# simone7monaco/NO-NODE-comparison

Hardware: NVIDIA B200
Metric: train trajectories/s (EGNO 20-body, fwd+bwd+Adam) (higher is better)
Workload: dtype f32

## Files before the change

include/nbody_b200.h:

```cpp
#ifndef NBODY_B200_H
#define NBODY_B200_H

#include <stdint.h>

#ifdef __cplusplus
extern "C" {
#endif

#define NB_HIDDEN 64
#define NB_MAX_EDGE_FEA 4
#define NB_MAX_T 16
#define NB_MAX_NODES 100

#define NB_OK 0
#define NB_ERR_INVALID (-1)
#define NB_ERR_CUDA (-2)

typedef struct NbEgnoConfig {
  int32_t B;
  int32_t N;
  int32_t T;
  int32_t n_layers;
  int32_t num_modes;
  int32_t in_node_nf;
  int32_t in_edge_nf;
  int32_t time_emb_dim;
  int32_t use_time_conv;
  int32_t num_inputs;
} NbEgnoConfig;

typedef struct NbSegnoConfig {
  int32_t B;
  int32_t N;
  int32_t T;
  int32_t in_node_nf;
  int32_t in_edge_nf;
  int32_t recurrent;
  float coords_weight;
  int32_t h_given;
} NbSegnoConfig;

int nb_version(void);
const char* nb_last_error(void);

int64_t nb_egno_param_count(const NbEgnoConfig* cfg);
int64_t nb_segno_param_count(const NbSegnoConfig* cfg);

#define NB_WS_FORWARD_INFER 0
#define NB_WS_BACKWARD 1
#define NB_WS_FORWARD_TRAIN 2
int64_t nb_egno_saved_floats(const NbEgnoConfig* cfg);
int64_t nb_egno_workspace_floats(const NbEgnoConfig* cfg, int mode);
int64_t nb_segno_saved_floats(const NbSegnoConfig* cfg);
int64_t nb_segno_workspace_floats(const NbSegnoConfig* cfg, int mode);

int nb_egno_forward(const NbEgnoConfig* cfg, const float* params, const float* x, const float* nodes,
                    const float* edge_fea, const float* v, const float* loc_mean, const int64_t* timesteps_out,
                    const int64_t* timesteps_in, float* x_out, float* v_out, float* h_out, float* saved,
                    float* workspace, void* stream);

int nb_egno_backward(const NbEgnoConfig* cfg, const float* params, const float* nodes, const float* edge_fea,
                     const float* loc_mean, const int64_t* timesteps_out, const int64_t* timesteps_in,
                     const float* saved, const float* g_x_out, const float* g_v_out, const float* g_h_out,
                     float* grad_params, float* g_x_in, float* g_v_in, float* workspace, void* stream);

int nb_segno_forward(const NbSegnoConfig* cfg, const float* params, const float* his, const float* x, const float* v,
                     const float* edge_attr, float* x_out, float* h_out, float* v_out, float* saved,
                     float* workspace, void* stream);

int nb_segno_backward(const NbSegnoConfig* cfg, const float* params, const float* his, const float* edge_attr,
                      const float* saved, const float* g_x_out, const float* g_h_out, const float* g_v_out,
                      float* grad_params, float* g_x_in, float* g_v_in, float* g_h_in, float* workspace, void* stream);

int nb_segno_embed_forward(const NbSegnoConfig* cfg, const float* params, int64_t rows, const float* his, float* h,
                           void* stream);
int64_t nb_segno_embed_backward_workspace_floats(const NbSegnoConfig* cfg, int64_t rows);
int nb_segno_embed_backward(const NbSegnoConfig* cfg, int64_t rows, const float* his, const float* g_h, float* grad_params,
                            float* workspace, void* stream);
int nb_segno_merge_forward(int32_t mode, int64_t n, int32_t L, int32_t frame, const float* h_all, const float* x_all,
                           const float* v_all, const float* h_int, const float* x_int, const float* v_int,
                           const float* attn_params, float* h_out, float* x_out, float* v_out, float* alpha, void* stream);
int64_t nb_segno_merge_backward_workspace_floats(int64_t n);
int nb_segno_merge_backward(int32_t mode, int64_t n, int32_t L, int32_t frame, const float* h_all, const float* x_all,
                            const float* v_all, const float* h_int, const float* x_int, const float* v_int,
                            const float* attn_params, const float* alpha, const float* g_h, const float* g_x,
                            const float* g_v, float* g_h_all, float* g_x_all, float* g_v_all, float* g_h_int,
                            float* g_x_int, float* g_v_int, float* g_attn, int32_t accumulate, float* workspace,
                            void* stream);
int nb_accumulate(int64_t n, float* dst, const float* src, void* stream);

int nb_check_canonical_edges(const int64_t* row, const int64_t* col, int64_t n_edges, int32_t B, int32_t N,
                             int32_t* flag_dev, void* stream);


int nb_egcl_edge_forward(int32_t n_gt, int32_t B, int32_t N, int32_t n_edge_fea, int32_t clamp_per_edge,
                         const float* x, const float* P, const float* Q, const float* edge_fea, const float* w1,
                         int32_t ldw1, int32_t col_rad, int32_t col_ef, const float* W2, const float* b2,
                         const float* W3, const float* b3, const float* w4, const float* b4, float* M, float* Fsum,
                         void* stream);

int64_t nb_egcl_edge_backward_workspace_floats(int32_t n_gt, int32_t N);
int nb_egcl_edge_backward(int32_t n_gt, int32_t B, int32_t N, int32_t n_edge_fea, int32_t clamp_per_edge,
                          const float* x, const float* P, const float* Q, const float* edge_fea, const float* w1,
                          int32_t ldw1, int32_t col_rad, int32_t col_ef, const float* W2, const float* b2,
                          const float* W3, const float* b3, const float* w4, const float* b4, const float* gM,
                          const float* gFsum, float* gP, float* gQ, float* gx, float* gw, float* workspace,
                          void* stream);

long long nb_launch_count(void);
#define NB_PROFILE_CATEGORIES 8
int nb_profile_enable(int enable);
int nb_profile_read(double* ms , long long* counts );

int nb_set_edge_impl(int impl);
int nb_get_edge_impl(void);
int nb_set_node_impl(int impl);
int nb_get_node_impl(void);
int nb_set_node_fused(int on);
int nb_get_node_fused(void);
int nb_set_segno_fused(int on);
int nb_get_segno_fused(void);

int nb_nbody_features(int32_t B, int32_t N, int32_t with_charge, const float* loc, const float* vel, const float* charges,
                      const float* edge_attr_o, float* nodes, float* loc_mean, float* edge_attr, void* stream);
int nb_nbody_energy(int32_t kind, int32_t F, int32_t B, int32_t N, float G, const float* loc, const float* vel,
                    const float* charges, float* energy, void* stream);

int64_t nb_traj_mse_workspace_floats(int32_t T);
int nb_traj_mse(int32_t T, int64_t rows, int32_t target_layout, int32_t only_first, const float* pred, const float* target,
                float* losses, float* loss, float* grad, float* workspace, void* stream);

int nb_sim_charged(int32_t B, int32_t N, int32_t T, int32_t sample_freq, double dt, double strength, double max_force,
                   double box_size, const double* loc0, const double* vel0, const double* charges, double* loc, double* vel,
                   void* stream);
int nb_sim_gravity(int32_t B, int32_t N, int32_t T, int32_t sample_freq, double dt, double G, double softening,
                   const double* pos0, const double* vel0, const double* mass, double* pos, double* vel, double* force,
                   void* stream);

int nb_adam_step(int64_t n, float* params, const float* grads, float* exp_avg, float* exp_avg_sq, float* step,
                 int32_t tick, double lr, double beta1, double beta2, double eps, double weight_decay, double grad_scale,
                 void* stream);
int nb_adam_step_peers(int64_t n, float* params, const void* const* peer_grads, int32_t npeer, float* exp_avg,
                       float* exp_avg_sq, float* step, int32_t tick, double lr, double beta1, double beta2, double eps,
                       double weight_decay, double grad_scale, void* stream);

int nb_tc_selftest(int32_t mode, const float* A, const float* W, float* out, void* stream);

int nb_silu_selftest(int64_t n, const float* x, float* out_mufu, float* out_fma, void* stream);

#ifdef __cplusplus
}
#endif
#endif
```

no-node-comparison_b200/_cabi.py:

```python
from __future__ import annotations

import ctypes as C

c_f = C.c_void_p


class NbEgnoConfig(C.Structure):
    _fields_ = [("B", C.c_int32), ("N", C.c_int32), ("T", C.c_int32), ("n_layers", C.c_int32),
                ("num_modes", C.c_int32), ("in_node_nf", C.c_int32), ("in_edge_nf", C.c_int32),
                ("time_emb_dim", C.c_int32), ("use_time_conv", C.c_int32), ("num_inputs", C.c_int32)]


class NbSegnoConfig(C.Structure):
    _fields_ = [("B", C.c_int32), ("N", C.c_int32), ("T", C.c_int32), ("in_node_nf", C.c_int32),
                ("in_edge_nf", C.c_int32), ("recurrent", C.c_int32), ("coords_weight", C.c_float),
                ("h_given", C.c_int32)]


EXPORTS = {
    "nb_version": (C.c_int, []),
    "nb_last_error": (C.c_char_p, []),
    "nb_egno_param_count": (C.c_int64, [C.POINTER(NbEgnoConfig)]),
    "nb_segno_param_count": (C.c_int64, [C.POINTER(NbSegnoConfig)]),
    "nb_egno_saved_floats": (C.c_int64, [C.POINTER(NbEgnoConfig)]),
    "nb_egno_workspace_floats": (C.c_int64, [C.POINTER(NbEgnoConfig), C.c_int]),
    "nb_segno_saved_floats": (C.c_int64, [C.POINTER(NbSegnoConfig)]),
    "nb_segno_workspace_floats": (C.c_int64, [C.POINTER(NbSegnoConfig), C.c_int]),
    "nb_egno_forward": (C.c_int, [C.POINTER(NbEgnoConfig)] + [c_f] * 14),
    "nb_egno_backward": (C.c_int, [C.POINTER(NbEgnoConfig)] + [c_f] * 15),
    "nb_segno_forward": (C.c_int, [C.POINTER(NbSegnoConfig)] + [c_f] * 11),
    "nb_segno_backward": (C.c_int, [C.POINTER(NbSegnoConfig)] + [c_f] * 13),
    "nb_segno_embed_forward": (C.c_int, [C.POINTER(NbSegnoConfig), c_f, C.c_int64, c_f, c_f, c_f]),
    "nb_segno_embed_backward_workspace_floats": (C.c_int64, [C.POINTER(NbSegnoConfig), C.c_int64]),
    "nb_segno_embed_backward": (C.c_int, [C.POINTER(NbSegnoConfig), C.c_int64] + [c_f] * 5),
    "nb_segno_merge_forward": (C.c_int, [C.c_int32, C.c_int64, C.c_int32, C.c_int32] + [c_f] * 12),
    "nb_segno_merge_backward_workspace_floats": (C.c_int64, [C.c_int64]),
    "nb_segno_merge_backward": (C.c_int, [C.c_int32, C.c_int64, C.c_int32, C.c_int32] + [c_f] * 18 + [C.c_int32, c_f, c_f]),
    "nb_accumulate": (C.c_int, [C.c_int64, c_f, c_f, c_f]),
    "nb_check_canonical_edges": (C.c_int, [c_f, c_f, C.c_int64, C.c_int32, C.c_int32, c_f, c_f]),
    "nb_egcl_edge_forward": (C.c_int, [C.c_int32] * 5 + [c_f] * 5 + [C.c_int32] * 3 + [c_f] * 9),
    "nb_egcl_edge_backward_workspace_floats": (C.c_int64, [C.c_int32, C.c_int32]),
    "nb_egcl_edge_backward": (C.c_int, [C.c_int32] * 5 + [c_f] * 5 + [C.c_int32] * 3 + [c_f] * 14),
    "nb_nbody_features": (C.c_int, [C.c_int32] * 3 + [c_f] * 8),
    "nb_nbody_energy": (C.c_int, [C.c_int32] * 4 + [C.c_float] + [c_f] * 5),
    "nb_sim_charged": (C.c_int, [C.c_int32] * 4 + [C.c_double] * 4 + [c_f] * 6),
    "nb_sim_gravity": (C.c_int, [C.c_int32] * 4 + [C.c_double] * 3 + [c_f] * 7),
    "nb_traj_mse_workspace_floats": (C.c_int64, [C.c_int32]),
    "nb_traj_mse": (C.c_int, [C.c_int32, C.c_int64, C.c_int32, C.c_int32] + [c_f] * 7),
    "nb_adam_step": (C.c_int, [C.c_int64] + [c_f] * 5 + [C.c_int32] + [C.c_double] * 6 + [c_f]),
    "nb_adam_step_peers": (C.c_int, [C.c_int64, c_f, C.POINTER(C.c_void_p), C.c_int32] + [c_f] * 3 + [C.c_int32] + [C.c_double] * 6 + [c_f]),
    "nb_launch_count": (C.c_longlong, []),
    "nb_profile_enable": (C.c_int, [C.c_int]),
    "nb_profile_read": (C.c_int, [C.POINTER(C.c_double), C.POINTER(C.c_longlong)]),
    "nb_set_edge_impl": (C.c_int, [C.c_int]),
    "nb_set_node_impl": (C.c_int, [C.c_int]),
    "nb_get_node_impl": (C.c_int, []),
    "nb_set_node_fused": (C.c_int, [C.c_int]),
    "nb_get_node_fused": (C.c_int, []),
    "nb_set_segno_fused": (C.c_int, [C.c_int]),
    "nb_get_segno_fused": (C.c_int, []),
    "nb_get_edge_impl": (C.c_int, []),
    "nb_tc_selftest": (C.c_int, [C.c_int32, c_f, c_f, c_f, c_f]),
    "nb_silu_selftest": (C.c_int, [C.c_int64, c_f, c_f, c_f, c_f]),
}


def declare(lib: C.CDLL) -> C.CDLL:
    for name, (res, args) in EXPORTS.items():
        fn = getattr(lib, name)
        fn.restype = res
        fn.argtypes = args
    return lib
```

no-node-comparison_b200/csrc/nb_edge_sel.cuh:

```cuda
#pragma once
#ifndef NB_EMU
#include "nb_edge.cuh"
#include "nb_tc.cuh"
#include "nb_edge_tc.cuh"

#define NB_SEL_MAX_GN 27
#define NB_SEL_XC0 54

struct NbSelUnit {
  int R;
  int gt0;
  int recv0, nrecv;
  int send0, nsend;
  int RC;
  int I0, J0;
  bool first_j, last_j;
  bool first_i, last_i;
};
template <bool BLK>
__device__ __forceinline__ NbSelUnit nb_sel_unit(const NbEdgeGeom& g, int uo, int sub) {
  NbSelUnit U;
  if (!BLK) {
    U.gt0 = uo * g.G;
    const int ngt = min(g.G, g.NGT - U.gt0);
// ... 338 lines not shown
                 sNl = nb_smem_u32(Nl), sFh = nb_smem_u32(Fh), sFl = nb_smem_u32(Fl), sW2h = nb_smem_u32(W2h),
                 sW2l = nb_smem_u32(W2l), sW3h = nb_smem_u32(W3h), sW3l = nb_smem_u32(W3l);
  const float b4 = __ldg(a.w.b4);
  uint32_t phase = 0;

  const int n_outer = BLK ? g.NGT : g.n_units, n_sub = BLK ? g.nI * g.nJ : 1;
  for (int uo = blockIdx.x; uo < n_outer; uo += gridDim.x)
  for (int sub = 0; sub < n_sub; ++sub) {
    const NbSelUnit U = nb_sel_unit<BLK>(g, uo, sub);
    const int R = U.R;
    {
      const int n3r = U.nrecv * 3, n3 = n3r + (BLK ? U.nsend * 3 : 0);
      const int t_x = tid + (U.first_j ? 0 : n3r);
      float xv = 0.f;
      if (t_x < n3) xv = t_x < n3r ? __ldg(a.x + (int64_t)U.recv0 * 3 + t_x) : __ldg(a.x + (int64_t)U.send0 * 3 + (t_x - n3r));
      nb_sel_stage_unit(Nh, Nl, a.P, a.Q, U, tid, NB_THREADS, U.first_j);
      if (t_x < n3) {
        if (t_x < n3r) xs[t_x] = xv;
        else xq[t_x - n3r] = xv;
      }
    }
    const float* xsnd = BLK ? xq : xs;
    __syncthreads();

    for (int r0 = 0; r0 < R; r0 += NB_TILE) {
      float dx = 0.f, dy = 0.f, dz = 0.f, r2 = 0.f;
      float e[NB_MAX_EF];
#pragma unroll
      for (int f = 0; f < NB_MAX_EF; ++f) e[f] = 0.f;
      int li = 0, lj = 0, gt = 0, rem = 0;
      const bool valid = nb_sel_row<BLK>(g, U, rowinfo, r0 + row, li, lj, gt, rem);
      if (valid) {
        dx = xs[li * 3 + 0] - xsnd[lj * 3 + 0];
        dy = xs[li * 3 + 1] - xsnd[lj * 3 + 1];
        dz = xs[li * 3 + 2] - xsnd[lj * 3 + 2];
        r2 = dx * dx + dy * dy + dz * dz;
        const int64_t eoff = ((int64_t)nb_ef_graph(g, gt) * g.EPG + rem) * g.nef;
#pragma unroll
        for (int f = 0; f < NB_MAX_EF; ++f)
          if (f < g.nef) e[f] = __ldg(a.ef + eoff + f);
      }
      if (r0 > 0) {
        nb_mbar_wait(bar, phase);
        phase ^= 1;
        nb_tc_fence_after();
      }
      nb_sel_write_row(Sel, row, hf, valid, li, U.RC + lj, r2, e);
      nb_fence_async_smem();
      nb_tc_fence_before();
      __syncthreads();
      if (NB_ISSUER(0)) {
        nb_tc_fence_after();
        nb_issue_gather(tm, sSel, sNh, sNl, 4, idesc_gat, 0u);
        nb_mma_commit(bar);
      }
      nb_mbar_wait(bar, phase);
      phase ^= 1;
      nb_tc_fence_after();
      {
        float v[32];
        nb_tmem_ld32(tm_mine, v);
#pragma unroll
        for (int i = 0; i < 32; ++i) v[i] = NB_FWD_SILU(i, v[i]);
        nb_store32_ta(nullptr, nullptr, row, hf, v, ta_hm, ta_lm);
        nb_tmem_st_wait();
      }
      nb_tc_fence_before();
      __syncthreads();
      if (NB_ISSUER(0)) {
        nb_tc_fence_after();
        nb_issue_w3_ta(tm, ta_h, ta_l, sW2h, sW2l, false, idesc_fwd, 0u);
        nb_mma_commit(bar);
      }
      nb_mbar_wait(bar, phase);
      phase ^= 1;
      nb_tc_fence_after();
      {
        float v[32];
        nb_tmem_ld32(tm_mine, v);
#pragma unroll
        for (int i = 0; i < 32; ++i) v[i] = NB_FWD_SILU(i, v[i] + vb2[cb + i]);
        nb_store32_ta(Th, Tl, row, hf, v, ta_hm, ta_lm);
        nb_tmem_st_wait();
      }
      nb_fence_async_smem();
      nb_tc_fence_before();
      __syncthreads();
      if (NB_ISSUER(0)) {
        nb_tc_fence_after();
        nb_issue_w3_ta(tm, ta_h, ta_l, sW3h, sW3l, false, idesc_fwd, 0u);
        nb_mma_commit(bar);
        nb_issue_scatter(tm + 64, sSel, sTh, sTl, idesc_sc, (r0 > 0 || !U.first_j) ? 1u : 0u);
      }
      nb_mbar_wait(bar, phase);
      phase ^= 1;
      nb_tc_fence_after();
      {
        float v[32];
        nb_tmem_ld32(tm_mine, v);
        float cp = 0.f;
#pragma unroll
        for (int i = 0; i < 32; ++i) cp = fmaf(vw4[cb + i], NB_FWD_SILU(i, v[i] + vb3[cb + i]), cp);
        cpart[hf * NB_TILE + row] = cp;
      }
      nb_tc_fence_before();
      __syncthreads();
      if (hf == 0) {
        float c = cpart[row] + cpart[NB_TILE + row] + b4;
        float fx = dx * c, fy = dy * c, fz = dz * c;
        if (g.clamp_edge) {
          fx = fminf(fmaxf(fx, -100.f), 100.f);
          fy = fminf(fmaxf(fy, -100.f), 100.f);
          fz = fminf(fmaxf(fz, -100.f), 100.f);
        }
        const uint32_t px = nb_pack_split(fx), py = nb_pack_split(fy), pz = nb_pack_split(fz);
        *reinterpret_cast<uint4*>(Fh + row * 16) = make_uint4((px & 0xffffu) | (py << 16), pz & 0xffffu, 0u, 0u);
        *reinterpret_cast<uint4*>(Fl + row * 16) = make_uint4((px >> 16) | (py & 0xffff0000u), pz >> 16, 0u, 0u);
      }
      nb_fence_async_smem();
      __syncthreads();
      if (NB_ISSUER(0)) {
        nb_tc_fence_after();
        nb_issue_scatter8(tm + 128, sSel, sFh, sFl, idesc_sc8, (r0 > 0 || !U.first_j) ? 1u : 0u);
        nb_mma_commit(bar);
      }
    }
    nb_mbar_wait(bar, phase);
    phase ^= 1;
    nb_tc_fence_after();
    if (U.last_j) {
      const int nl = 16 * q + lane;
      float v[32];
      nb_tmem_ld32(tm + ((uint32_t)(32 * q) << 16) + 64 + (uint32_t)cb, v);
      if (lane < 16 && nl < U.nrecv) {
        float* dst = a.M + (int64_t)(U.recv0 + nl) * NB_H + cb;
#pragma unroll
        for (int k = 0; k < 8; ++k) nb_st4(dst + 4 * k, make_float4(v[4 * k], v[4 * k + 1], v[4 * k + 2], v[4 * k + 3]));
      }
      float f4[4];
      nb_tmem_ld4(tm + ((uint32_t)(32 * q) << 16) + 128, f4);
      if (hf == 0 && lane < 16 && nl < U.nrecv) {
        float* dst = a.Fsum + (int64_t)(U.recv0 + nl) * 3;
        dst[0] = f4[0];
        dst[1] = f4[1];
        dst[2] = f4[2];
      }
    }
    nb_tc_fence_before();
    __syncthreads();
  }
  nb_tc_fence_before();
  __syncthreads();
  if (warp == 0) nb_tmem_dealloc(tm, NB_SF_TMEM_COLS);
}

#define NB_SB_THREADS 512
#define NB_SB_W 0
#define NB_SB_TZ (4 * NB_TC_TILE_BYTES(64))
#define NB_SB_TM (NB_SB_TZ + 2 * NB_TC_TILE_BYTES(128))
#define NB_SB_TG (NB_SB_TM + 2 * NB_TC_TILE_BYTES(128))
#define NB_SB_SEL (NB_SB_TG + 2 * NB_TC_TILE_BYTES(128))
#define NB_SB_NT (NB_SB_SEL + NB_TC_TILE_BYTES(128))
#define NB_SB_GM (NB_SB_NT + 2 * NB_TC_TILE_BYTES(64))
#define NB_SB_ONES (NB_SB_GM + 2 * NB_TC_TILE_BYTES(64))
#define NB_SB_RG (NB_SB_ONES + NB_TILE * 16)
#define NB_SB_FL (NB_SB_RG + 2 * NB_TILE * 16)
#define NB_SB_NFLOAT (4 * NB_H + 4 * NB_TILE + 3 * 32 * 3 + 10 * NB_H + NB_H * 4 + NB_MAX_EF * NB_H)
#define NB_SB_QLD 68
#define NB_EDGE_BWD_SEL_SMEM(RU) (NB_SB_FL + NB_SB_NFLOAT * 4 + (RU) * 4 + 64 + 1024)
#define NB_SB_GXACC(N) (((N) * 3 + 3) / 4 * 4)
#define NB_EDGE_BWD_SEL_BLK_EXTRA(N) ((32 * NB_H + (N) * NB_H + NB_SB_GXACC(N)) * 4)
#define NB_SB_TMEM_COLS 512

__device__ __forceinline__ void nb_tmem_ld16(uint32_t taddr, float (&v)[16]) {
  uint32_t r[16];
  asm volatile(
      "tcgen05.ld.sync.aligned.32x32b.x16.b32 "
      "{%0, %1, %2, %3, %4, %5, %6, %7, %8, %9, %10, %11, %12, %13, %14, %15}, [%16];"
      : "=r"(r[0]), "=r"(r[1]), "=r"(r[2]), "=r"(r[3]), "=r"(r[4]), "=r"(r[5]), "=r"(r[6]), "=r"(r[7]), "=r"(r[8]),
        "=r"(r[9]), "=r"(r[10]), "=r"(r[11]), "=r"(r[12]), "=r"(r[13]), "=r"(r[14]), "=r"(r[15])
      : "r"(taddr)
      : "memory");
  asm volatile("tcgen05.wait::ld.sync.aligned;" ::: "memory");
#pragma unroll
  for (int i = 0; i < 16; ++i) v[i] = __uint_as_float(r[i]);
}
__device__ __forceinline__ void nb_tmem_st16_nowait(uint32_t taddr, const float (&v)[16]) {
  asm volatile(
      "tcgen05.st.sync.aligned.32x32b.x16.b32 [%0], "
      "{%1, %2, %3, %4, %5, %6, %7, %8, %9, %10, %11, %12, %13, %14, %15, %16};" ::"r"(taddr),
      "r"(__float_as_uint(v[0])), "r"(__float_as_uint(v[1])), "r"(__float_as_uint(v[2])), "r"(__float_as_uint(v[3])),
      "r"(__float_as_uint(v[4])), "r"(__float_as_uint(v[5])), "r"(__float_as_uint(v[6])), "r"(__float_as_uint(v[7])),
      "r"(__float_as_uint(v[8])), "r"(__float_as_uint(v[9])), "r"(__float_as_uint(v[10])), "r"(__float_as_uint(v[11])),
      "r"(__float_as_uint(v[12])), "r"(__float_as_uint(v[13])), "r"(__float_as_uint(v[14])), "r"(__float_as_uint(v[15]))
      : "memory");
}

__device__ __forceinline__ void nb_issue_wgrad(uint32_t tmem_w, uint32_t tmem_b, uint32_t g_hi, uint32_t g_lo, uint32_t a_hi,
                                               uint32_t a_lo, uint32_t ones, uint32_t idesc_wg, uint32_t idesc_bs,
                                               uint32_t acc0) {
  uint32_t acc = acc0;
#pragma unroll
  for (int pass = 0; pass < 3; ++pass) {
    const uint32_t ga = nb_desc_lo_mn(pass == 1 ? g_lo : g_hi);
    const uint32_t ab = nb_desc_lo_mn(pass == 2 ? a_lo : a_hi);
#pragma unroll
    for (int s = 0; s < 8; ++s) {
      nb_mma2(tmem_w, ga + NB_KSTEP_MN * s, NB_DESC_HI_SW128, ab + NB_KSTEP_MN * s, NB_DESC_HI_SW128, idesc_wg, acc);
      acc = 1u;
    }
  }
  acc = acc0;
  const uint32_t ob = nb_desc_lo_n8(ones);
#pragma unroll
  for (int pass = 0; pass < 2; ++pass) {
    const uint32_t ga = nb_desc_lo_mn(pass ? g_lo : g_hi);
#pragma unroll
    for (int s = 0; s < 8; ++s) {
      nb_mma2(tmem_b, ga + NB_KSTEP_MN * s, NB_DESC_HI_SW128, ob + NB_KSTEP_N8 * s, NB_DESC_HI_NOSW, idesc_bs, acc);
      acc = 1u;
    }
  }
}

#ifdef NB_STAGE_CLOCKS
__device__ long long nb_dbg_clk[32];
#define NB_CLK(i)                                   \
  if (dbg_on) {                                     \
    const long long t_now = clock64();              \
    dbg_acc[i] += t_now - dbg_last;                 \
    dbg_last = t_now;                               \
  }
#else
#define NB_CLK(i)
#endif

__device__ __forceinline__ void nb_issue_wgrad_fold(uint32_t tmem_w, uint32_t g_hi, uint32_t g_lo, uint32_t a_hi, uint32_t a_lo,
                                                    uint32_t lbo, uint32_t idesc64, uint32_t idesc72, uint32_t acc0) {
  uint32_t acc = acc0;
  const uint32_t b72 = ((a_hi >> 4) & 0x3FFFu) | ((lbo >> 4) << 16);
#pragma unroll
  for (int pass = 0; pass < 3; ++pass) {
    const uint32_t ga = nb_desc_lo_mn(pass == 1 ? g_lo : g_hi);
    const uint32_t ab = pass == 2 ? nb_desc_lo_mn(a_lo) : b72;
#pragma unroll
    for (int s = 0; s < 8; ++s) {
      nb_mma2(tmem_w, ga + NB_KSTEP_MN * s, NB_DESC_HI_SW128, ab + NB_KSTEP_MN * s, NB_DESC_HI_SW128, pass == 2 ? idesc64 : idesc72, acc);
      acc = 1u;
    }
  }
}
__device__ __forceinline__ void nb_issue_scatter_fold(uint32_t tmem_d, uint32_t sel, uint32_t v_hi, uint32_t v_lo, uint32_t lbo_hi,
                                                      uint32_t lbo_lo, uint32_t idesc72, uint32_t acc0) {
  uint32_t acc = acc0;
  const uint32_t a = nb_desc_lo_mn(sel);
#pragma unroll
  for (int pass = 0; pass < 2; ++pass) {
    const uint32_t b = (((pass ? v_lo : v_hi) >> 4) & 0x3FFFu) | (((pass ? lbo_lo : lbo_hi) >> 4) << 16);
#pragma unroll
    for (int s = 0; s < 8; ++s) {
      nb_mma2(tmem_d, a + NB_KSTEP_MN * s, NB_DESC_HI_SW128, b + NB_KSTEP_MN * s, NB_DESC_HI_SW128, idesc72, acc);
      acc = 1u;
    }
  }
}
#define NB_SB_ONES64_BYTES NB_TC_TILE_BYTES(128)

template <bool BLK>
__global__ void __launch_bounds__(NB_SB_THREADS, 1) k_edge_bwd_sel(NbEdgeBwdArgs a) {
  NB_PDL_ENTER();
#ifdef NB_STAGE_CLOCKS
  __shared__ long long dbg_acc[32];
  const bool dbg_on = blockIdx.x == 0 && threadIdx.x == 0;
  const long long dbg_t0 = clock64();
  unsigned long long dbg_g0;
  asm volatile("mov.u64 %0, %%globaltimer;" : "=l"(dbg_g0));
  long long dbg_last = 0;
  if (dbg_on) {
    for (int i = 0; i < 32; ++i) dbg_acc[i] = 0;
    dbg_last = clock64();
  }
#endif
  extern __shared__ __align__(1024) unsigned char nb_smraw[];
  unsigned char* base = nb_smraw + ((1024u - (nb_smem_u32(nb_smraw) & 1023u)) & 1023u);
  unsigned char* W2h = base + NB_SB_W;
  unsigned char* W2l = W2h + NB_TC_TILE_BYTES(64);
  unsigned char* W3h = W2l + NB_TC_TILE_BYTES(64);
  unsigned char* W3l = W3h + NB_TC_TILE_BYTES(64);
  unsigned char* Tzh = base + NB_SB_TZ;
  unsigned char* Tzl = Tzh + NB_TC_TILE_BYTES(128);
  unsigned char* Tmh = base + NB_SB_TM;
  unsigned char* Tml = Tmh + NB_TC_TILE_BYTES(128);
  unsigned char* Tgh = base + NB_SB_TG;
  unsigned char* Tgl = Tgh + NB_TC_TILE_BYTES(128);
  unsigned char* Sel = base + NB_SB_SEL;
  float* Pf = reinterpret_cast<float*>(base + NB_SB_NT);
  float* Qf = Pf + (BLK ? a.g.IB : a.g.G * a.g.N) * NB_H;
  float* gMs = reinterpret_cast<float*>(base + NB_SB_GM);
  unsigned char* ones = base + NB_SB_ONES;
  unsigned char* RGh = base + NB_SB_RG;
  unsigned char* RGl = RGh + NB_TILE * 16;
  float* scratch = reinterpret_cast<float*>(Tzh);
  constexpr bool FOLD = !BLK;
  unsigned char* ones64 = base + NB_SB_FL;
  float* fl = reinterpret_cast<float*>(base + NB_SB_FL + (FOLD ? NB_SB_ONES64_BYTES : 0));
  float* vb2 = fl;
// ... 542 lines not shown
```

no-node-comparison_b200/csrc/nbody_b200.cu:

```cuda
#include <math.h>
#include <stdarg.h>
#include <stdio.h>
#include <string.h>

#include "nb_common.cuh"
#include "nb_node.cuh"
#include "nb_spectral.cuh"
#include "nb_rollout.cuh"
#include "nb_sim.cuh"
#include "nb_edge.cuh"
#include "nb_tc.cuh"
#include "nb_edge_tc.cuh"
#include "nb_edge_sel.cuh"
#include "nb_node_tc.cuh"
#include "nb_segno_fused.cuh"
#include "nb_merge.cuh"
#include "nb_egno_node.cuh"
#include <cstdlib>

#define NB_LAUNCH_COUNTED(...)                             \
  do {                                                     \
    __atomic_fetch_add(&g_launches, 1LL, __ATOMIC_RELAXED); \
    NB_LAUNCH(__VA_ARGS__);                                \
  } while (0)
// ... 401 lines not shown
  int grid = imin(cdiv(maxrows, NB_TILE), wgrad_grid_cap());
#ifndef NB_EMU
  if (g_node_impl == 1) {
    static int ctas = 0;
    if (!ctas) { const char* e = getenv("NB_B200_WGRAD_CTAS"); ctas = (e && e[0] >= '1' && e[0] <= '3') ? e[0] - '0' : 2; }
    int per_job = ctas * nb_num_sms() / wb.njobs;
    if (per_job < 16) per_job = 16;
    if (per_job > nb_num_sms()) per_job = nb_num_sms();
    grid = imin(cdiv(maxrows, NB_TILE), per_job);
  }
#endif
  const int64_t need = (int64_t)wb.njobs * grid * NB_WGRAD_PLEN;
  if (g_q.pused + need > g_q.pcap) NB_TRY(q_flush_fin(st));
  if (need > g_q.pcap) { nb_set_error("partial-sum workspace too small"); return NB_ERR_INVALID; }
  for (int j = 0; j < wb.njobs; ++j) {
    wb.job[j].partial = g_q.pbase + g_q.pused;
    g_q.pused += (int64_t)grid * NB_WGRAD_PLEN;
  }
  bool wdone = false;
#ifndef NB_EMU
  if (g_node_impl == 1) {
    const size_t smem_tc = NB_WT_SMEM;
    NB_SET_SMEM(k_wgrad64_tc, smem_tc);
    int pi_tc = prof_begin(3, st);
    NB_LAUNCH_COUNTED(k_wgrad64_tc, dim3((unsigned)grid, (unsigned)wb.njobs), NB_THREADS, smem_tc, st, wb);
    prof_end(3, pi_tc, st);
    NB_TRY(nb_check_launch("k_wgrad64_tc"));
    wdone = true;
  }
#endif
  if (!wdone) {
    const size_t smem = 2 * NB_TILE * NB_LDA * sizeof(float);
    NB_SET_SMEM(k_wgrad64, smem);
    int pi = prof_begin(3, st);
    NB_LAUNCH_COUNTED(k_wgrad64, dim3((unsigned)grid, (unsigned)wb.njobs), NB_THREADS, smem, st, wb);
    prof_end(3, pi, st);
    NB_TRY(nb_check_launch("k_wgrad64"));
  }
  const int n = wb.njobs;
  wb.njobs = 0;
  for (int j = 0; j < n; ++j) {
    NbFinArgs f;
    memset(&f, 0, sizeof(f));
    const WgradFin& wf = g_q.wfin[j];
    f.partial = wb.job[j].partial; f.nparts = grid; f.plen = NB_WGRAD_PLEN; f.dst = wf.dst; f.accumulate = wf.accumulate;
    f.nseg = 0;
    f.seg[f.nseg++] = fseg(0, NB_H * NB_H, NB_H, wf.w_off, wf.so, wf.si);
    f.seg[f.nseg - 1].klimit = wf.klimit;
    if (wf.b_off >= 0) f.seg[f.nseg++] = fseg(NB_H * NB_H, NB_H, NB_H, wf.b_off, 0, 1);
    NB_TRY(launch_finalize(f, st));
  }
  return NB_OK;
}
static int q_flush(void* st) {
  NB_TRY(q_flush_wgrad(st));
  return q_flush_fin(st);
}

struct DeferState {
  bool on;
  int k;
  float* arena[2];
};
static bool defer_available() {
#ifndef NB_EMU
  static int off = -1;
  if (off < 0) { const char* e = getenv("NB_B200_WGRAD_DEFER"); off = (e && e[0] == '0') ? 1 : 0; }
  return !off && side_get() != nullptr;
#else
  return false;
#endif
}
static int defer_flush(DeferState& D, void* main_st) {
#ifndef NB_EMU
  if (D.on) {
    NbSide* x = side_get();
    cudaStream_t ms = (cudaStream_t)main_st;
    cudaEventRecord(x->fork2, ms);
    cudaStreamWaitEvent(x->s2, x->fork2, 0);
    NB_TRY(q_flush((void*)x->s2));
    cudaEventRecord(x->done2[D.k & 1], x->s2);
    if (D.k > 0) cudaStreamWaitEvent(ms, x->done2[(D.k - 1) & 1], 0);
    ++D.k;
    g_q.pbase = D.arena[D.k & 1];
    g_q.pused = 0;
    return nb_check_launch("deferred flush");
  }
#endif
  return q_flush(main_st);
}
static void defer_join(DeferState& D, void* main_st) {
#ifndef NB_EMU
  if (D.on && D.k > 0) cudaStreamWaitEvent((cudaStream_t)main_st, side_get()->done2[(D.k - 1) & 1], 0);
#else
  (void)D; (void)main_st;
#endif
}

static int wgrad_to(int rows, int npair, NbWgradPair p0, NbWgradPair p1, float* dst, int64_t w_off, int64_t so,
                    int64_t si, int64_t b_off, int accumulate, void* st, int klimit = 0) {
  if (rows <= 0) return NB_OK;
  if (g_q.wb.njobs == NB_MAX_WGRAD_JOBS) NB_TRY(q_flush_wgrad(st));
  NbWgradArgs a;
  memset(&a, 0, sizeof(a));
  a.rows = rows; a.npair = npair; a.pair[0] = p0; a.pair[1] = p1; a.colsum = b_off >= 0;
  WgradFin wf;
  wf.w_off = w_off; wf.so = so; wf.si = si; wf.b_off = b_off; wf.dst = dst; wf.accumulate = accumulate; wf.klimit = klimit;
  g_q.wfin[g_q.wb.njobs] = wf;
  g_q.wb.job[g_q.wb.njobs++] = a;
  return NB_OK;
}

static NbWgradPair wpair(const float* G, const float* A, int a_silu = 0, float scale = 1.f) {
  NbWgradPair p;
  p.G = G; p.ldg = NB_H; p.A = A; p.lda = NB_H; p.a_silu = a_silu; p.scale = scale;
  p.seg_rows = 0; p.seg_g = p.seg_a = 0;
  return p;
}
static NbWgradPair wpair_seg(const float* G, const float* A, int a_silu, int seg_rows, int64_t seg_g, int64_t seg_a) {
  NbWgradPair p = wpair(G, A, a_silu);
  p.seg_rows = seg_rows; p.seg_g = seg_g; p.seg_a = seg_a;
  return p;
}

static int ew_grid(int64_t n) { return imin(cdiv(n, 256), 8 * nb_num_sms()); }

static NbEdgeGeom edge_geom(int n_gt, int B, int N, int nef, int clamp_edge) {
  NbEdgeGeom g;
  memset(&g, 0, sizeof(g));
  g.N = N; g.EPG = N * (N - 1); g.NGT = n_gt; g.B = B; g.nef = nef; g.clamp_edge = clamp_edge;
  int G = NB_TILE / g.EPG;
  if (G < 1) G = 1;
  if (G * N > 128) G = 128 / N;
  if (G < 1) G = 1;
  g.G = G;
  g.n_units = (int)cdiv(n_gt, G);
  return g;
}

#ifdef NB_EMU
static int g_edge_impl = 0;
#else
static int g_edge_impl = 2;
#endif
extern "C" int nb_set_edge_impl(int impl) {
#ifdef NB_EMU
  if (impl != 0) { nb_set_error("the host emulator only runs the SIMT edge tiles"); return NB_ERR_INVALID; }
#endif
  if (impl < 0 || impl > 2) { nb_set_error("edge impl must be 0 (SIMT), 1 (tcgen05) or 2 (tcgen05 + selector MMAs)"); return NB_ERR_INVALID; }
  g_edge_impl = impl;
  return NB_OK;
}
extern "C" int nb_get_edge_impl(void) { return g_edge_impl; }

#ifndef NB_EMU
static bool sel_geom(NbEdgeGeom& g) {
  if (g.N > NB_SEL_MAX_GN) {
    if (g.N > 255) return false;
    g.blk = 1;
    int best = 1 << 30;
    for (int ib = 1; ib <= 32; ++ib) {
      int jb = NB_TILE / ib;
      if (jb > 32) jb = 32;
      if (jb > g.N) jb = g.N;
      if (ib + jb > NB_SEL_XC0 || jb < 1) continue;
      const int tiles = (int)(cdiv(g.N, ib) * cdiv(g.N, jb));
      if (tiles < best) { best = tiles; g.IB = ib; g.JB = jb; }
    }
    g.nI = (int)cdiv(g.N, g.IB);
    g.nJ = (int)cdiv(g.N, g.JB);
    g.G = 1;
    g.n_units = g.NGT;
    return true;
  }
  g.blk = 0; g.nI = g.nJ = g.IB = g.JB = 0;
  int G = NB_TILE / g.EPG;
  if (G > NB_SEL_MAX_GN / g.N) G = NB_SEL_MAX_GN / g.N;
  if (G < 1) G = 1;
  g.G = G;
  g.n_units = (int)cdiv(g.NGT, G);
  return true;
}
#endif

static int launch_edge_fwd(NbEdgeFwdArgs& a, void* st) {
#ifndef NB_EMU
  if (g_edge_impl == 2) {
    if (!sel_geom(a.g)) { nb_set_error("selector edge kernels support at most 255 nodes per graph (N=%d)", a.g.N); return NB_ERR_INVALID; }
    const size_t smem_sel = NB_EDGE_FWD_SEL_SMEM(a.g.blk ? 0 : a.g.G * a.g.EPG);
    int grid_sel = imin(a.g.n_units, 2 * nb_num_sms());
    int pi_sel = prof_begin(0, st);
    if (a.g.blk) {
      NB_SET_SMEM(k_edge_fwd_sel<true>, smem_sel);
      NB_LAUNCH_COUNTED(k_edge_fwd_sel<true>, (unsigned)grid_sel, NB_THREADS, smem_sel, st, a);
    } else {
      NB_SET_SMEM(k_edge_fwd_sel<false>, smem_sel);
      NB_LAUNCH_COUNTED(k_edge_fwd_sel<false>, (unsigned)grid_sel, NB_THREADS, smem_sel, st, a);
    }
    prof_end(0, pi_sel, st);
    return nb_check_launch("k_edge_fwd_sel");
  }
  if (g_edge_impl >= 1) {
    const size_t smem_tc = NB_EDGE_FWD_TC_SMEM;
    NB_SET_SMEM(k_edge_fwd_tc, smem_tc);
    int grid_tc = imin(a.g.n_units, 3 * nb_num_sms());
    int pi_tc = prof_begin(0, st);
    NB_LAUNCH_COUNTED(k_edge_fwd_tc, (unsigned)grid_tc, NB_THREADS, smem_tc, st, a);
    prof_end(0, pi_tc, st);
    return nb_check_launch("k_edge_fwd_tc");
  }
#endif
  const size_t smem = NB_EDGE_FWD_SMEM_FLOATS * sizeof(float);
  NB_SET_SMEM(k_edge_fwd, smem);
  int grid = imin(a.g.n_units, 3 * nb_num_sms());
  int pi = prof_begin(0, st);
  NB_LAUNCH_COUNTED(k_edge_fwd, (unsigned)grid, NB_THREADS, smem, st, a);
  prof_end(0, pi, st);
  return nb_check_launch("k_edge_fwd");
}

struct EdgeGradDst {
  int64_t w1, b_unused, W2, b2, W3, b3, w4, b4;
  int ldw1, col_rad, col_ef;
};

static int edge_bwd_finalize(float* partial, int nparts, int nef, float* dst, const EdgeGradDst& d, int accumulate, void* st) {
  NbFinArgs f;
  memset(&f, 0, sizeof(f));
  f.partial = partial; f.nparts = nparts; f.plen = NB_EB_PLEN; f.dst = dst; f.accumulate = accumulate;
  f.nseg = 0;
  f.seg[f.nseg++] = fseg(NB_EB_GW2, NB_H * NB_H, NB_H, d.W2, NB_H, 1);
  f.seg[f.nseg++] = fseg(NB_EB_GW3, NB_H * NB_H, NB_H, d.W3, NB_H, 1);
  f.seg[f.nseg++] = fseg(NB_EB_GB2, NB_H, NB_H, d.b2, 0, 1);
  f.seg[f.nseg++] = fseg(NB_EB_GB3, NB_H, NB_H, d.b3, 0, 1);
  f.seg[f.nseg++] = fseg(NB_EB_GW4, NB_H, NB_H, d.w4, 0, 1);
  f.seg[f.nseg++] = fseg(NB_EB_GWR, NB_H, 1, d.w1 + d.col_rad, d.ldw1, 0);
  f.seg[f.nseg++] = fseg(NB_EB_GWE, nef * NB_H, NB_H, d.w1 + d.col_ef, 1, d.ldw1);
  f.seg[f.nseg++] = fseg(NB_EB_GB4, 1, 1, d.b4, 0, 0);
  return launch_finalize(f, st);
}

static int launch_edge_bwd(NbEdgeBwdArgs& a, float* dst, const EdgeGradDst& d, int accumulate, void* st,
                           float** run_base = nullptr, int* run_parts = nullptr) {
  bool use_sel = false;
#ifndef NB_EMU
  if (g_edge_impl == 2) {
    if (!sel_geom(a.g)) { nb_set_error("selector edge kernels support at most 255 nodes per graph (N=%d)", a.g.N); return NB_ERR_INVALID; }
    use_sel = true;
  }
#endif
  int grid = imin(a.g.n_units, use_sel ? nb_num_sms() : edge_bwd_grid_cap());
  if (run_base && *run_parts > 0 && g_q.pused + ((int64_t)grid * NB_EB_PLEN + 63) / 64 * 64 > g_q.pcap) {
    NB_TRY(edge_bwd_finalize(*run_base, *run_parts, a.g.nef, dst, d, accumulate, st));
    NB_TRY(q_flush(st));
    *run_parts = 0;
  }
  float* partial = q_alloc((int64_t)grid * NB_EB_PLEN, st);
  if (!partial) { nb_set_error("partial-sum workspace too small"); return NB_ERR_INVALID; }
  a.partial = partial;
  if (run_base) {
    if (*run_parts == 0) *run_base = partial;
    else if (partial != *run_base + (int64_t)*run_parts * NB_EB_PLEN) { nb_set_error("edge backward partial slices are not contiguous"); return NB_ERR_INVALID; }
  }
  bool done = false;
#ifndef NB_EMU
  if (use_sel) {
    const size_t smem_sel = NB_EDGE_BWD_SEL_SMEM(a.g.blk ? 0 : a.g.G * a.g.EPG) +
                            (a.g.blk ? NB_EDGE_BWD_SEL_BLK_EXTRA(a.g.N) : NB_SB_ONES64_BYTES);
    int pi_sel = prof_begin(1, st);
    if (a.g.blk) {
      NB_SET_SMEM(k_edge_bwd_sel<true>, smem_sel);
      NB_LAUNCH_COUNTED(k_edge_bwd_sel<true>, (unsigned)grid, NB_SB_THREADS, smem_sel, st, a);
    } else {
      NB_SET_SMEM(k_edge_bwd_sel<false>, smem_sel);
      NB_LAUNCH_COUNTED(k_edge_bwd_sel<false>, (unsigned)grid, NB_SB_THREADS, smem_sel, st, a);
    }
    prof_end(1, pi_sel, st);
    NB_TRY(nb_check_launch("k_edge_bwd_sel"));
    done = true;
  } else if (g_edge_impl >= 1) {
    const size_t smem_tc = NB_EDGE_BWD_TC_SMEM(a.g.G * a.g.N);
    NB_SET_SMEM(k_edge_bwd_tc, smem_tc);
    int pi_tc = prof_begin(1, st);
    NB_LAUNCH_COUNTED(k_edge_bwd_tc, (unsigned)grid, NB_THREADS, smem_tc, st, a);
    prof_end(1, pi_tc, st);
    NB_TRY(nb_check_launch("k_edge_bwd_tc"));
    done = true;
  }
#endif
  if (!done) {
    const size_t smem = NB_EDGE_BWD_SMEM_FLOATS(a.g.G * a.g.N) * sizeof(float);
    NB_SET_SMEM(k_edge_bwd, smem);
    int pi = prof_begin(1, st);
    NB_LAUNCH_COUNTED(k_edge_bwd, (unsigned)grid, NB_THREADS, smem, st, a);
    prof_end(1, pi, st);
    NB_TRY(nb_check_launch("k_edge_bwd"));
  }
  if (run_base) {
    *run_parts += grid;
    return NB_OK;
  }
  return edge_bwd_finalize(partial, grid, a.g.nef, dst, d, accumulate, st);
}

static int make_twiddle(int T, int modes, NbTwiddle* tw) {
  if (T < 1 || T > NB_MAX_T || modes < 1 || modes > T / 2 + 1) {
    nb_set_error("unsupported temporal conv: T=%d (<= %d), modes=%d (<= T/2+1)", T, NB_MAX_T, modes);
    return NB_ERR_INVALID;
  }
  memset(tw, 0, sizeof(*tw));
  tw->T = T;
  tw->modes = modes;
  tw->nyq = (T % 2 == 0 && modes - 1 >= T / 2) ? T / 2 : -1;
  if (T == 1) tw->nyq = -1;
  tw->ncoef = 1 + 2 * (modes - 1);
  for (int m = 0; m < modes; ++m)
    for (int t = 0; t < T; ++t) {
      double th = 2.0 * M_PI * (double)((m * t) % T) / (double)T;
      tw->c[m][t] = (float)cos(th);
      tw->s[m][t] = (m == 0 || m == tw->nyq) ? 0.f : (float)sin(th);
    }
  return NB_OK;
}

#define NB_MAX_LAYERS 32
struct EgnoLayerOff {
  int64_t e_w1, e_b1, e_w2, e_b2, c_w1, c_b1, c_w2, c_b2, v_w1, v_b1, v_w2, v_b2, n_w1, n_b1, n_w2, n_b2, tc, tcx;
};
struct EgnoLayout {
  int F, E;
  int64_t emb_w, emb_b, total;
  EgnoLayerOff L[NB_MAX_LAYERS];
};

static int egno_validate(const NbEgnoConfig* c) {
  if (!c) { nb_set_error("null config"); return NB_ERR_INVALID; }
  if (c->B < 1 || c->N < 2 || c->N > NB_MAX_NODES) { nb_set_error("unsupported B=%d N=%d (2 <= N <= %d)", c->B, c->N, NB_MAX_NODES); return NB_ERR_INVALID; }
  if (c->n_layers < 1 || c->n_layers > NB_MAX_LAYERS) { nb_set_error("unsupported n_layers=%d", c->n_layers); return NB_ERR_INVALID; }
  if (c->T < 1 || c->T > NB_MAX_T) { nb_set_error("unsupported num_timesteps=%d (<= %d)", c->T, NB_MAX_T); return NB_ERR_INVALID; }
  if (c->use_time_conv && (c->num_modes < 1 || c->num_modes > c->T / 2 + 1)) { nb_set_error("num_modes=%d must be in [1, T/2+1] for T=%d", c->num_modes, c->T); return NB_ERR_INVALID; }
  if (c->in_edge_nf < 0 || c->in_edge_nf > NB_MAX_EDGE_FEA) { nb_set_error("unsupported in_edge_nf=%d", c->in_edge_nf); return NB_ERR_INVALID; }
// ... 1528 lines not shown
```

Baseline: 79520.

## Add warp-specialized three-group edge forward kernel with mbarrier-pipelined tcgen05 MMAs

Adds a new edge-forward kernel for graphs whose edge count spans several tiles. A dedicated issuer warp drives tcgen05 MMAs for three independent 128-row consumer groups, each with its own tensor-memory accumulator region, using mbarriers instead of block-wide syncs. The next unit's node tables and coordinates are double-buffered and staged while the current unit's tiles are processed. The aim is to overlap SiLU epilogues and tensor-core work across tiles, at the cost of more shared memory, one CTA per SM and a more complex synchronization scheme. It is on by default behind a new runtime toggle.

```diff
diff --git a/include/nbody_b200.h b/include/nbody_b200.h
--- a/include/nbody_b200.h
+++ b/include/nbody_b200.h
@@ -114,6 +114,8 @@
 
 int nb_set_edge_impl(int impl);
 int nb_get_edge_impl(void);
+int nb_set_edge_fwd3(int on);
+int nb_get_edge_fwd3(void);
 int nb_set_node_impl(int impl);
 int nb_get_node_impl(void);
 int nb_set_node_fused(int on);
diff --git a/no-node-comparison_b200/_cabi.py b/no-node-comparison_b200/_cabi.py
--- a/no-node-comparison_b200/_cabi.py
+++ b/no-node-comparison_b200/_cabi.py
@@ -60,6 +60,8 @@
     "nb_set_segno_fused": (C.c_int, [C.c_int]),
     "nb_get_segno_fused": (C.c_int, []),
     "nb_get_edge_impl": (C.c_int, []),
+    "nb_set_edge_fwd3": (C.c_int, [C.c_int]),
+    "nb_get_edge_fwd3": (C.c_int, []),
     "nb_tc_selftest": (C.c_int, [C.c_int32, c_f, c_f, c_f, c_f]),
     "nb_silu_selftest": (C.c_int, [C.c_int64, c_f, c_f, c_f, c_f]),
 }
diff --git a/no-node-comparison_b200/csrc/nb_edge_sel.cuh b/no-node-comparison_b200/csrc/nb_edge_sel.cuh
--- a/no-node-comparison_b200/csrc/nb_edge_sel.cuh
+++ b/no-node-comparison_b200/csrc/nb_edge_sel.cuh
@@ -514,6 +514,309 @@
   nb_tc_fence_before();
   __syncthreads();
   if (warp == 0) nb_tmem_dealloc(tm, NB_SF_TMEM_COLS);
+}
+
+#define NB_F3_GROUPS 3
+#define NB_F3_THREADS (128 * NB_F3_GROUPS + 32)
+#define NB_F3_ISSUER_WARP (4 * NB_F3_GROUPS)
+#define NB_F3_W 0
+#define NB_F3_NT (4 * NB_TC_TILE_BYTES(64))
+#define NB_F3_GRP (NB_F3_NT + 4 * NB_TC_TILE_BYTES(64))
+#define NB_F3_GRP_BYTES (3 * NB_TC_TILE_BYTES(128) + 2 * NB_TILE * 16)
+#define NB_F3_FL (NB_F3_GRP + NB_F3_GROUPS * NB_F3_GRP_BYTES)
+#define NB_F3_NFLOAT (3 * NB_H + 2 * 32 * 3)
+#define NB_EDGE_FWD_SEL3_SMEM(RU) (NB_F3_FL + NB_F3_NFLOAT * 4 + (RU) * 4 + 16 * 8 + 1024)
+#define NB_F3_TMEM_COLS 512
+#define NB_F3_TM_M 384
+#define NB_F3_TM_F 448
+
+__device__ __forceinline__ void nb_named_sync(int id, int nthreads) {
+  asm volatile("bar.sync %0, %1;" ::"r"(id), "r"(nthreads) : "memory");
+}
+__device__ __forceinline__ void nb_mbar_arrive(uint64_t* bar) {
+  asm volatile("mbarrier.arrive.shared::cta.b64 _, [%0];" ::"r"(nb_smem_u32(bar)) : "memory");
+}
+
+__global__ void __launch_bounds__(NB_F3_THREADS, 1) k_edge_fwd_sel3(NbEdgeFwdArgs a) {
+  NB_PDL_ENTER();
+  extern __shared__ __align__(1024) unsigned char nb_smraw[];
+  unsigned char* base = nb_smraw + ((1024u - (nb_smem_u32(nb_smraw) & 1023u)) & 1023u);
+  unsigned char* W2h = base + NB_F3_W;
+  unsigned char* W2l = W2h + NB_TC_TILE_BYTES(64);
+  unsigned char* W3h = W2l + NB_TC_TILE_BYTES(64);
+  unsigned char* W3l = W3h + NB_TC_TILE_BYTES(64);
+  unsigned char* NT = base + NB_F3_NT;
+  float* fl = reinterpret_cast<float*>(base + NB_F3_FL);
+  float* vb2 = fl;
+  float* vb3 = vb2 + NB_H;
+  float* vw4 = vb3 + NB_H;
+  float* xsb = vw4 + NB_H;
+  uint32_t* rowinfo = reinterpret_cast<uint32_t*>(xsb + 2 * 32 * 3);
+  const NbEdgeGeom g = a.g;
+  const int RU = g.G * g.EPG;
+  uint64_t* bars = reinterpret_cast<uint64_t*>(rowinfo + RU + (RU & 1));
+  uint64_t* ready = bars;
+  uint64_t* done = bars + 3;
+  uint64_t* ntfull = bars + 6;
+  uint64_t* accfree = bars + 8;
+  uint32_t* tmem_slot = reinterpret_cast<uint32_t*>(bars + 9);
+  constexpr int NC = 128 * NB_F3_GROUPS;
+
+  const int tid = threadIdx.x, warp = tid >> 5, lane = tid & 31;
+  const int grp = warp >> 2, q = warp & 3;
+  const int row = 32 * q + lane;
+
+  if (tid < NB_THREADS) {
+    nb_tc_stage_weight(W2h, W2l, a.w.W2, tid);
+    nb_tc_stage_weight(W3h, W3l, a.w.W3, tid);
+  }
+  for (int idx = tid; idx < 4 * NB_TC_TILE_BYTES(64) / 16; idx += NB_F3_THREADS)
+    reinterpret_cast<uint4*>(NT)[idx] = make_uint4(0u, 0u, 0u, 0u);
+  nb_sel_build_rowinfo(rowinfo, g, tid, NB_F3_THREADS);
+  if (tid < NB_H) {
+    vb2[tid] = __ldg(a.w.b2 + tid);
+    vb3[tid] = __ldg(a.w.b3 + tid);
+    vw4[tid] = __ldg(a.w.w4 + tid);
+  }
+  if (tid == 0) {
+    for (int i = 0; i < NB_F3_GROUPS; ++i) {
+      nb_mbar_init(ready + i, 1);
+      nb_mbar_init(done + i, 1);
+    }
+    nb_mbar_init(ntfull, NC);
+    nb_mbar_init(ntfull + 1, NC);
+    nb_mbar_init(accfree, 128);
+    nb_mbar_fence_init();
+  }
+  if (warp == 0) nb_tmem_alloc(tmem_slot, NB_F3_TMEM_COLS);
+  __syncthreads();
+  for (int idx = tid; idx < 2 * 10 * 8; idx += NB_F3_THREADS) {
+    const int b = idx / 80, k = (idx % 80) >> 3, j = idx & 7;
+    const int f = (k >> 1) - 1;
+    float v[8];
+#pragma unroll
+    for (int i = 0; i < 8; ++i) {
+      const int c = 8 * j + i;
+      v[i] = f < 0 ? __ldg(a.w.W1 + (int64_t)c * a.w.ldw1 + a.w.col_rad)
+                   : (f < g.nef ? __ldg(a.w.W1 + (int64_t)c * a.w.ldw1 + a.w.col_ef + f) : 0.f);
+    }
+    unsigned char* nh = NT + 2 * b * NB_TC_TILE_BYTES(64);
+    nb_tc_store8(nh, nh + NB_TC_TILE_BYTES(64), NB_SEL_XC0 + k, j, v);
+  }
+  if (blockIdx.x < g.n_units) {
+    const NbSelUnit U = nb_sel_unit<false>(g, blockIdx.x, 0);
+    nb_sel_stage_unit(NT, NT + NB_TC_TILE_BYTES(64), a.P, a.Q, U, tid, NB_F3_THREADS);
+    if (tid < U.nrecv * 3) xsb[tid] = __ldg(a.x + (int64_t)U.recv0 * 3 + tid);
+  }
+  nb_fence_async_smem();
+  nb_tc_fence_before();
+  __syncthreads();
+  nb_tc_fence_after();
+  const uint32_t tm = *tmem_slot;
+  const uint32_t idesc_fwd = nb_idesc_bf16(128, 64, 0, 0);
+  const uint32_t idesc_gat = nb_idesc_bf16(128, 64, 0, 1);
+  const uint32_t idesc_sc = nb_idesc_bf16(64, 64, 1, 1);
+  const uint32_t idesc_sc8 = nb_idesc_bf16(64, 8, 1, 1);
+
+  if (warp == NB_F3_ISSUER_WARP) {
+    if (nb_elect_one()) {
+      const uint32_t sW2h = nb_smem_u32(W2h), sW2l = nb_smem_u32(W2l), sW3h = nb_smem_u32(W3h), sW3l = nb_smem_u32(W3l);
+      const uint32_t sGrp = nb_smem_u32(base + NB_F3_GRP);
+      uint32_t ph_ready = 0;
+      int k = 0;
+      for (int uo = blockIdx.x; uo < g.n_units; uo += gridDim.x, ++k) {
+        const int ntl = (nb_sel_unit<false>(g, uo, 0).R + NB_TILE - 1) / NB_TILE;
+        const uint32_t sNh = nb_smem_u32(NT + 2 * (k & 1) * NB_TC_TILE_BYTES(64)), sNl = sNh + NB_TC_TILE_BYTES(64);
+        if (k > 0) nb_mbar_wait(ntfull + (k & 1), ((k - 1) >> 1) & 1);
+        for (int t0 = 0; t0 < ntl; t0 += NB_F3_GROUPS) {
+          const int ng = min(NB_F3_GROUPS, ntl - t0);
+#pragma unroll 1
+          for (int st = 0; st < 4; ++st)
+#pragma unroll 1
+            for (int gi = 0; gi < ng; ++gi) {
+              const uint32_t sSel = sGrp + gi * NB_F3_GRP_BYTES, sTh = sSel + NB_TC_TILE_BYTES(128),
+                             sTl = sTh + NB_TC_TILE_BYTES(128), sFh = sTl + NB_TC_TILE_BYTES(128), sFl = sFh + NB_TILE * 16;
+              const uint32_t tg = tm + 128u * gi;
+              const uint32_t acc = (t0 + gi > 0) ? 1u : 0u;
+              nb_mbar_wait(ready + gi, (ph_ready >> gi) & 1u);
+              ph_ready ^= 1u << gi;
+              nb_tc_fence_after();
+              if (st == 0) {
+                nb_issue_gather(tg, sSel, sNh, sNl, 4, idesc_gat, 0u);
+              } else if (st == 1) {
+                nb_issue_w3_ta(tg, tg + 64, tg + 96, sW2h, sW2l, false, idesc_fwd, 0u);
+              } else if (st == 2) {
+                nb_issue_w3_ta(tg, tg + 64, tg + 96, sW3h, sW3l, false, idesc_fwd, 0u);
+                nb_mma_commit(done + gi);
+                if (t0 + gi == 0 && k > 0) {
+                  nb_mbar_wait(accfree, (k - 1) & 1);
+                  nb_tc_fence_after();
+                }
+                nb_issue_scatter(tm + NB_F3_TM_M, sSel, sTh, sTl, idesc_sc, acc);
+                continue;
+              } else {
+                nb_issue_scatter8(tm + NB_F3_TM_F, sSel, sFh, sFl, idesc_sc8, acc);
+              }
+              nb_mma_commit(done + gi);
+            }
+        }
+      }
+    }
+    __syncwarp();
+  } else {
+    unsigned char* Sel = base + NB_F3_GRP + grp * NB_F3_GRP_BYTES;
+    unsigned char* Th = Sel + NB_TC_TILE_BYTES(128);
+    unsigned char* Tl = Th + NB_TC_TILE_BYTES(128);
+    unsigned char* Fh = Tl + NB_TC_TILE_BYTES(128);
+    unsigned char* Fl = Fh + NB_TILE * 16;
+    const uint32_t lq = (uint32_t)(32 * q) << 16;
+    const uint32_t tpre = tm + lq + 128u * grp;
+    const uint32_t ta_h = tpre + 64, ta_l = tpre + 96;
+    const float b4 = __ldg(a.w.b4);
+    uint32_t phase = 0;
+    bool pend = false;
+    int k = 0;
+    for (int uo = blockIdx.x; uo < g.n_units; uo += gridDim.x, ++k) {
+      const NbSelUnit U = nb_sel_unit<false>(g, uo, 0);
+      const int R = U.R, ntl = (R + NB_TILE - 1) / NB_TILE;
+      const int b = k & 1;
+      if (k > 0) nb_mbar_wait(ntfull + b, ((k - 1) >> 1) & 1);
+      const float* xs = xsb + b * 96;
+      for (int t = grp; t < ntl; t += NB_F3_GROUPS) {
+        const int r0 = t * NB_TILE;
+        float dx = 0.f, dy = 0.f, dz = 0.f, r2 = 0.f;
+        float e[NB_MAX_EF];
+#pragma unroll
+        for (int f = 0; f < NB_MAX_EF; ++f) e[f] = 0.f;
+        int li = 0, lj = 0, gt = 0, rem = 0;
+        const bool valid = nb_sel_row<false>(g, U, rowinfo, r0 + row, li, lj, gt, rem);
+        if (valid) {
+          dx = xs[li * 3 + 0] - xs[lj * 3 + 0];
+          dy = xs[li * 3 + 1] - xs[lj * 3 + 1];
+          dz = xs[li * 3 + 2] - xs[lj * 3 + 2];
+          r2 = dx * dx + dy * dy + dz * dz;
+          const int64_t eoff = ((int64_t)nb_ef_graph(g, gt) * g.EPG + rem) * g.nef;
+#pragma unroll
+          for (int f = 0; f < NB_MAX_EF; ++f)
+            if (f < g.nef) e[f] = __ldg(a.ef + eoff + f);
+        }
+        if (pend) {
+          nb_mbar_wait(done + grp, phase);
+          phase ^= 1;
+          nb_tc_fence_after();
+        }
+        nb_sel_write_row(Sel, row, 0, valid, li, U.RC + lj, r2, e);
+        nb_sel_write_row(Sel, row, 1, valid, li, U.RC + lj, r2, e);
+        nb_fence_async_smem();
+        nb_tc_fence_before();
+        nb_named_sync(1 + grp, 128);
+        if (row == 0) nb_mbar_arrive(ready + grp);
+        nb_mbar_wait(done + grp, phase);
+        phase ^= 1;
+        nb_tc_fence_after();
+#pragma unroll
+        for (int hf = 0; hf < 2; ++hf) {
+          float v[32];
+          nb_tmem_ld32(tpre + 32 * hf, v);
+#pragma unroll
+          for (int i = 0; i < 32; ++i) v[i] = NB_FWD_SILU(i, v[i]);
+          nb_store32_ta(nullptr, nullptr, row, hf, v, ta_h + 16 * hf, ta_l + 16 * hf);
+        }
+        nb_tmem_st_wait();
+        nb_tc_fence_before();
+        nb_named_sync(1 + grp, 128);
+        if (row == 0) nb_mbar_arrive(ready + grp);
+        if (t == grp && uo + (int)gridDim.x < g.n_units) {
+          const NbSelUnit Un = nb_sel_unit<false>(g, uo + gridDim.x, 0);
+          unsigned char* nh = NT + 2 * (b ^ 1) * NB_TC_TILE_BYTES(64);
+          const float xv = tid < Un.nrecv * 3 ? __ldg(a.x + (int64_t)Un.recv0 * 3 + tid) : 0.f;
+          nb_sel_stage_unit(nh, nh + NB_TC_TILE_BYTES(64), a.P, a.Q, Un, tid, NC);
+          if (tid < Un.nrecv * 3) xsb[(b ^ 1) * 96 + tid] = xv;
+          nb_fence_async_smem();
+          nb_mbar_arrive(ntfull + (b ^ 1));
+        }
+        nb_mbar_wait(done + grp, phase);
+        phase ^= 1;
+        nb_tc_fence_after();
+#pragma unroll
+        for (int hf = 0; hf < 2; ++hf) {
+          float v[32];
+          nb_tmem_ld32(tpre + 32 * hf, v);
+#pragma unroll
+          for (int i = 0; i < 32; ++i) v[i] = NB_FWD_SILU(i, v[i] + vb2[32 * hf + i]);
+          nb_store32_ta(Th, Tl, row, hf, v, ta_h + 16 * hf, ta_l + 16 * hf);
+        }
+        nb_tmem_st_wait();
+        nb_fence_async_smem();
+        nb_tc_fence_before();
+        nb_named_sync(1 + grp, 128);
+        if (row == 0) nb_mbar_arrive(ready + grp);
+        nb_mbar_wait(done + grp, phase);
+        phase ^= 1;
+        nb_tc_fence_after();
+        float cp[2];
+#pragma unroll
+        for (int hf = 0; hf < 2; ++hf) {
+          float v[32];
+          nb_tmem_ld32(tpre + 32 * hf, v);
+          cp[hf] = 0.f;
+#pragma unroll
+          for (int i = 0; i < 32; ++i) cp[hf] = fmaf(vw4[32 * hf + i], NB_FWD_SILU(i, v[i] + vb3[32 * hf + i]), cp[hf]);
+        }
+        {
+          const float c = cp[0] + cp[1] + b4;
+          float fx = dx * c, fy = dy * c, fz = dz * c;
+          if (g.clamp_edge) {
+            fx = fminf(fmaxf(fx, -100.f), 100.f);
+            fy = fminf(fmaxf(fy, -100.f), 100.f);
+            fz = fminf(fmaxf(fz, -100.f), 100.f);
+          }
+          const uint32_t px = nb_pack_split(fx), py = nb_pack_split(fy), pz = nb_pack_split(fz);
+          *reinterpret_cast<uint4*>(Fh + row * 16) = make_uint4((px & 0xffffu) | (py << 16), pz & 0xffffu, 0u, 0u);
+          *reinterpret_cast<uint4*>(Fl + row * 16) = make_uint4((px >> 16) | (py & 0xffff0000u), pz >> 16, 0u, 0u);
+        }
+        nb_fence_async_smem();
+        nb_tc_fence_before();
+        nb_named_sync(1 + grp, 128);
+        if (row == 0) nb_mbar_arrive(ready + grp);
+        pend = true;
+      }
+      if (grp == (ntl - 1) % NB_F3_GROUPS) {
+        nb_mbar_wait(done + grp, phase);
+        phase ^= 1;
+        pend = false;
+        nb_tc_fence_after();
+        const int nl = 16 * q + lane;
+#pragma unroll
+        for (int hf = 0; hf < 2; ++hf) {
+          float v[32];
+          nb_tmem_ld32(tm + lq + NB_F3_TM_M + 32 * hf, v);
+          if (lane < 16 && nl < U.nrecv) {
+            float* dst = a.M + (int64_t)(U.recv0 + nl) * NB_H + 32 * hf;
+#pragma unroll
+            for (int j = 0; j < 8; ++j) nb_st4(dst + 4 * j, make_float4(v[4 * j], v[4 * j + 1], v[4 * j + 2], v[4 * j + 3]));
+          }
+        }
+        float f4[4];
+        nb_tmem_ld4(tm + lq + NB_F3_TM_F, f4);
+        if (lane < 16 && nl < U.nrecv) {
+          float* dst = a.Fsum + (int64_t)(U.recv0 + nl) * 3;
+          dst[0] = f4[0];
+          dst[1] = f4[1];
+          dst[2] = f4[2];
+        }
+        nb_tc_fence_before();
+        nb_mbar_arrive(accfree);
+      }
+    }
+    if (pend) {
+      nb_mbar_wait(done + grp, phase);
+      nb_tc_fence_after();
+    }
+  }
+  nb_tc_fence_before();
+  __syncthreads();
+  if (warp == 0) nb_tmem_dealloc(tm, NB_F3_TMEM_COLS);
 }
 
 #define NB_SB_THREADS 512
diff --git a/no-node-comparison_b200/csrc/nbody_b200.cu b/no-node-comparison_b200/csrc/nbody_b200.cu
--- a/no-node-comparison_b200/csrc/nbody_b200.cu
+++ b/no-node-comparison_b200/csrc/nbody_b200.cu
@@ -577,6 +577,9 @@
   return NB_OK;
 }
 extern "C" int nb_get_edge_impl(void) { return g_edge_impl; }
+static int g_edge_fwd3 = 1;
+extern "C" int nb_set_edge_fwd3(int on) { g_edge_fwd3 = on ? 1 : 0; return NB_OK; }
+extern "C" int nb_get_edge_fwd3(void) { return g_edge_fwd3; }
 
 #ifndef NB_EMU
 static bool sel_geom(NbEdgeGeom& g) {
@@ -612,6 +615,15 @@
 #ifndef NB_EMU
   if (g_edge_impl == 2) {
     if (!sel_geom(a.g)) { nb_set_error("selector edge kernels support at most 255 nodes per graph (N=%d)", a.g.N); return NB_ERR_INVALID; }
+    if (g_edge_fwd3 && !a.g.blk && a.g.G == 1 && a.g.EPG > 2 * NB_TILE) {
+      const size_t smem3 = NB_EDGE_FWD_SEL3_SMEM(a.g.EPG);
+      const int grid3 = imin(a.g.n_units, nb_num_sms());
+      int pi3 = prof_begin(0, st);
+      NB_SET_SMEM(k_edge_fwd_sel3, smem3);
+      NB_LAUNCH_COUNTED(k_edge_fwd_sel3, (unsigned)grid3, NB_F3_THREADS, smem3, st, a);
+      prof_end(0, pi3, st);
+      return nb_check_launch("k_edge_fwd_sel3");
+    }
     const size_t smem_sel = NB_EDGE_FWD_SEL_SMEM(a.g.blk ? 0 : a.g.G * a.g.EPG);
     int grid_sel = imin(a.g.n_units, 2 * nb_num_sms());
     int pi_sel = prof_begin(0, st);
```

New measurement: 82450 (median of 6 runs). +3.7%, better.
